# yanielc/medical-vision-textural-bias

Hardware: AMD Instinct MI355X
Metric: BraTS 4ch 240^3 vols/sec filtered+train-step @1/2/4/8 GPU; filter HBM GB/s (higher is better)
Workload: dtype f32

## Files before the change

medical-vision-textural-bias_amd/csrc/conv_wgrad.hip:

```cpp
#include <hip/hip_runtime.h>

#include <cstdlib>

#include "conv_host.h"
#include "split_bf16.h"
#include "texbias.h"

namespace {

typedef float f32x4 __attribute__((ext_vector_type(4)));

constexpr int NT = 256;
constexpr int LDS_FLOATS = 78 * 1024 / 4;
constexpr int kSlack = 16;

struct WgArgs {
  const float* G;
  const float* X;
  float* dW;
  int M, Cc, Do, Ho, Wo, Di, Hi, Wi;
  int YB, YR, Wo4, XP, PG, PC, ncc, ctiles, nyb, xcols;
  int64_t nchunks;
};

// ... 732 lines not shown
  }
#pragma unroll
  for (int j = 0; j < NGL; ++j) {
    const int i = tid + NT * j;
    const int q = i % Wo4, t = i / Wo4, yy = t % YB, m = t / YB;
    const bool ok = m < mv && y0 + yy < Ho;
    gg[j] = ok ? (int)(((int64_t)m * Do) * oplane / 4 + ((y0 + yy) * Wo + 4 * q) / 4) : -1;
    gl[j] = m * a.MS + yy * Wo + 4 * q;
  }
  const int64_t iplane4 = iplane / 4, oplane4 = oplane / 4;
  float4 rx0[NXL], rx1[NXL], rg[NGL];
  auto load_x = [&](int zi, float4 (&rx)[NXL]) {
    const bool in = zi >= 0 && zi < Di;
    const float4* src = reinterpret_cast<const float4*>(Xb) + (int64_t)(in ? zi : 0) * iplane4;
#pragma unroll
    for (int j = 0; j < NXL; ++j) rx[j] = src[xg[j] < 0 ? 0 : xg[j]];
  };
  auto store_x = [&](int zi, const float4 (&rx)[NXL]) {
    float* d = xsl + ((zi + 5) % 5) * XS;
    const bool in = zi >= 0 && zi < Di;
#pragma unroll
    for (int j = 0; j < NXL; ++j)
      if (xg[j] >= 0) {
        const float4 v = in ? rx[j] : make_float4(0.f, 0.f, 0.f, 0.f);
        float2* p = reinterpret_cast<float2*>(d + xl[j]);
        p[0] = make_float2(v.x, v.y);
        p[1] = make_float2(v.z, v.w);
      }
  };
  auto load_g = [&](int z) {
#pragma unroll
    for (int j = 0; j < NGL; ++j) {
      rg[j] = (reinterpret_cast<const float4*>(Gb) + (int64_t)z * oplane4)[gg[j] < 0 ? 0 : gg[j]];
    }
  };
  auto store_g = [&](int z) {
    float* d = gsl + (z & 1) * GS;
#pragma unroll
    for (int j = 0; j < NGL; ++j)
      if (gg[j] >= 0) {
        float2* p = reinterpret_cast<float2*>(d + gl[j]);
        p[0] = make_float2(rg[j].x, rg[j].y);
        p[1] = make_float2(rg[j].z, rg[j].w);
      }
  };
  __syncthreads();
  load_x(2 * z0 - 1, rx0);
  store_x(2 * z0 - 1, rx0);
  load_x(2 * z0, rx0);
  load_x(2 * z0 + 1, rx1);
  load_g(z0);

  const int li = lane & 15, lk = lane >> 4;
  const int mtl = wave & 1, par = wave >> 1;
  const int aoff = (16 * mtl + li) * a.MS + lk;
  const int boff = li * a.RX + 2 * lk + 1;
  f32x4 acc[27];
#pragma unroll
  for (int j = 0; j < 27; ++j) acc[j] = f32x4{0.f, 0.f, 0.f, 0.f};
  for (int z = z0; z < z1; ++z) {
    store_x(2 * z, rx0);
    store_x(2 * z + 1, rx1);
    store_g(z);
    __syncthreads();
    load_x(2 * z + 2, rx0);
    load_x(2 * z + 3, rx1);
    load_g(z + 1 < z1 ? z + 1 : z);
    const float* ga = gsl + (z & 1) * GS + aoff;
    const float* xp[3] = {xsl + ((2 * z - 1 + 5) % 5) * XS + boff, xsl + ((2 * z) % 5) * XS + boff,
                          xsl + ((2 * z + 1) % 5) * XS + boff};
    const int nk = YB * Wo4;
    auto ld = [&](int k, float& av, float (&bv)[27]) {
      const int kk = k < nk ? k : nk - 1;
      const int yy = YB == 1 ? 0 : (kk >= Wo4 ? 1 : 0), x0 = 4 * (kk - yy * Wo4);
      av = ga[yy * Wo + x0];
#pragma unroll
      for (int tz = 0; tz < 3; ++tz)
#pragma unroll
        for (int ty = 0; ty < 3; ++ty)
#pragma unroll
          for (int tx = 0; tx < 3; ++tx) bv[tz * 9 + ty * 3 + tx] = xp[tz][(2 * yy + ty) * a.PX + 2 * x0 + tx];
    };
    auto mm = [&](float av, const float (&bv)[27]) {
#pragma unroll
      for (int t = 0; t < 27; ++t) acc[t] = __builtin_amdgcn_mfma_f32_16x16x4f32(av, bv[t], acc[t], 0, 0, 0);
    };
    if (par < nk) {
      float a0, a1, b0[27], b1[27];
      ld(par, a0, b0);
      int k = par;
      for (; k + P < nk; k += 2 * P) {
        ld(k + P, a1, b1);
        mm(a0, b0);
        ld(k + 2 * P, a0, b0);
        mm(a1, b1);
      }
      if (k < nk) mm(a0, b0);
    }
  }
  float* red = smem;
#pragma unroll
  for (int src = P - 1; src >= 1; --src) {
    __syncthreads();
    if (par == src) {
#pragma unroll
      for (int j = 0; j < 27; ++j)
#pragma unroll
        for (int rr = 0; rr < 4; ++rr) red[((mtl * 27 + j) * 4 + rr) * 64 + lane] = acc[j][rr];
    }
    __syncthreads();
    if (par == 0) {
#pragma unroll
      for (int j = 0; j < 27; ++j)
#pragma unroll
        for (int rr = 0; rr < 4; ++rr) acc[j][rr] += red[((mtl * 27 + j) * 4 + rr) * 64 + lane];
    }
  }
  if (par == 0) {
    const int c = li;
    float* pt = a.part ? a.part + ((int64_t)blockIdx.y * gridDim.x + blockIdx.x) * (32 * 16 * 27) : nullptr;
#pragma unroll
    for (int j = 0; j < 27; ++j)
#pragma unroll
      for (int rr = 0; rr < 4; ++rr) {
        const int m = 16 * mtl + lk * 4 + rr;
        if (pt) pt[(m * 16 + c) * 27 + j] = acc[j][rr];
        else if (m < mv && c < cv) atomicAdd(&a.dW[((int64_t)(m0 + m) * a.Cc + (c0 + c)) * 27 + j], acc[j][rr]);
      }
  }
}


struct Zf2Args {
  const float* G;
  const float* X;
  float* dW;
  float* part;
  int N, M, Cc, Do, Ho, Wo, Di, Hi, Wi;
  int YB, nyb, ZS, zlen;
  int MS, RX, PX;
  int mtiles;
};

template <int YB, int MT, int WV, int NW>
__global__ __launch_bounds__(64 * NW) void k_conv3d_wgrad_zf2(Zf2Args a) {
  constexpr int NT = 64 * NW;
  constexpr int NXR = 2 * YB + 1;
  extern __shared__ __attribute__((aligned(16))) float smem[];
  const int tid = (int)threadIdx.x, lane = tid & 63;
  const int wave = __builtin_amdgcn_readfirstlane(tid >> 6);
  const int Wo = a.Wo, Ho = a.Ho, Do = a.Do, Hi = a.Hi, Wi = a.Wi, Di = a.Di, Cc = a.Cc;
  const int GS = 16 * MT * a.MS, XS = Cc * a.RX;
  float* gsl = smem;
  float* xsl = smem + 2 * GS;
  int b = (int)blockIdx.x;
  const int zs = b % a.ZS;
  b /= a.ZS;
  const int yb = b % a.nyb, n = b / a.nyb;
  const int mt = (int)blockIdx.y;
  const int m0 = 16 * MT * mt, mv = min(16 * MT, a.M - m0);
  const int y0 = yb * YB;
  const int z0 = zs * a.zlen, z1 = min(Do, z0 + a.zlen);
  for (int i = tid; i < 2 * GS + 5 * XS; i += NT) smem[i] = 0.f;
  const int64_t iplane = (int64_t)Hi * Wi, oplane = (int64_t)Ho * Wo;
  const float* Gb = a.G + ((int64_t)n * a.M + m0) * Do * oplane;
  const float* Xb = a.X + (int64_t)n * Cc * Di * iplane;
  const int Wi4 = Wi >> 2, Wo4 = Wo >> 2;
  constexpr int NXL = (5 * NXR * 2 * WV + NT - 1) / NT, NGL = (16 * MT * YB * WV + NT - 1) / NT;
  int xg[NXL], xl[NXL], gg[NGL], gl[NGL];
#pragma unroll
  for (int j = 0; j < NXL; ++j) {
    const int i = tid + NT * j;
    const int q = i % Wi4, t = i / Wi4, r = t % NXR, c = t / NXR;
    const int yi = 2 * y0 - 1 + r;
    const bool ok = c < Cc && yi >= 0 && yi < Hi;
    xg[j] = ok ? (int)(((int64_t)c * Di) * iplane / 4 + (yi * Wi + 4 * q) / 4) : -1;
    xl[j] = c * a.RX + r * a.PX + 2 + 4 * q;
  }
#pragma unroll
  for (int j = 0; j < NGL; ++j) {
    const int i = tid + NT * j;
    const int q = i % Wo4, t = i / Wo4, yy = t % YB, m = t / YB;
    const int y = y0 + yy;
    const bool ok = m < mv && y < Ho;
    gg[j] = ok ? (int)(((int64_t)m * Do) * oplane / 4 + (y * Wo + 4 * q) / 4) : -1;
    gl[j] = m * a.MS + yy * Wo + 4 * q;
  }
  const int64_t iplane4 = iplane / 4, oplane4 = oplane / 4;
  float4 rx0[NXL], rx1[NXL], rg[NGL];
  auto load_x = [&](int zi, float4 (&rx)[NXL]) {
    const bool in = zi >= 0 && zi < Di;
    const float4* src = reinterpret_cast<const float4*>(Xb) + (int64_t)(in ? zi : 0) * iplane4;
#pragma unroll
    for (int j = 0; j < NXL; ++j) rx[j] = src[xg[j] < 0 ? 0 : xg[j]];
  };
  auto store_x = [&](int zi, const float4 (&rx)[NXL]) {
    float* d = xsl + ((zi + 5) % 5) * XS;
    const bool in = zi >= 0 && zi < Di;
#pragma unroll
    for (int j = 0; j < NXL; ++j)
      if (xg[j] >= 0) {
        const float4 v = in ? rx[j] : make_float4(0.f, 0.f, 0.f, 0.f);
        float2* p = reinterpret_cast<float2*>(d + xl[j]);
        p[0] = make_float2(v.x, v.y);
        p[1] = make_float2(v.z, v.w);
      }
  };
  auto load_g = [&](int z) {
#pragma unroll
    for (int j = 0; j < NGL; ++j) {
      rg[j] = (reinterpret_cast<const float4*>(Gb) + (int64_t)z * oplane4)[gg[j] < 0 ? 0 : gg[j]];
    }
  };
  auto store_g = [&](int z) {
    float* d = gsl + (z & 1) * GS;
#pragma unroll
    for (int j = 0; j < NGL; ++j)
      if (gg[j] >= 0) {
        float2* p = reinterpret_cast<float2*>(d + gl[j]);
        p[0] = make_float2(rg[j].x, rg[j].y);
        p[1] = make_float2(rg[j].z, rg[j].w);
      }
  };
  __syncthreads();
  load_x(2 * z0 - 1, rx0);
  store_x(2 * z0 - 1, rx0);
  load_x(2 * z0, rx0);
  load_x(2 * z0 + 1, rx1);
  load_g(z0);

  const int li = lane & 15, lk = lane >> 4;
  const int bc = li < 3 * Cc ? li / 3 : 0, btx = li < 3 * Cc ? li - 3 * (li / 3) : 0;
  const int boff = bc * a.RX + btx + 2 * lk + 1;
  f32x4 acc[MT][9];
#pragma unroll
  for (int t = 0; t < MT; ++t)
#pragma unroll
    for (int j = 0; j < 9; ++j) acc[t][j] = f32x4{0.f, 0.f, 0.f, 0.f};
  for (int z = z0; z < z1; ++z) {
    store_x(2 * z, rx0);
    store_x(2 * z + 1, rx1);
    store_g(z);
    __syncthreads();
    load_x(2 * z + 2, rx0);
    load_x(2 * z + 3, rx1);
    load_g(z + 1 < z1 ? z + 1 : z);
    const float* ga = gsl + (z & 1) * GS + li * a.MS + lk;
    const float* xp[3] = {xsl + ((2 * z - 1 + 5) % 5) * XS + boff, xsl + ((2 * z) % 5) * XS + boff,
                          xsl + ((2 * z + 1) % 5) * XS + boff};
    const int np = YB >= NW ? 1 : NW / YB, yy0 = YB >= NW ? wave : wave % YB, part = YB >= NW ? 0 : wave / YB;
    const int kb = (Wo4 * part) / np, ke = (Wo4 * (part + 1)) / np;
    auto ld = [&](int yy, int k, float (&av)[MT], float (&bv)[9]) {
      const int x0 = 4 * (k < ke ? k : ke - 1);
#pragma unroll
      for (int t = 0; t < MT; ++t) av[t] = ga[t * 16 * a.MS + yy * Wo + x0];
#pragma unroll
      for (int tz = 0; tz < 3; ++tz)
#pragma unroll
        for (int ty = 0; ty < 3; ++ty) bv[tz * 3 + ty] = xp[tz][(2 * yy + ty) * a.PX + 2 * x0];
    };
    auto mm = [&](const float (&av)[MT], const float (&bv)[9]) {
#pragma unroll
      for (int t = 0; t < MT; ++t)
#pragma unroll
        for (int j = 0; j < 9; ++j) acc[t][j] = __builtin_amdgcn_mfma_f32_16x16x4f32(av[t], bv[j], acc[t][j], 0, 0, 0);
    };
    for (int yy = yy0; yy < YB; yy += NW) {
      if (kb >= ke) break;
      float a0[MT], a1[MT], b0[9], b1[9];
      ld(yy, kb, a0, b0);
      int k = kb;
      for (; k + 1 < ke; k += 2) {
        ld(yy, k + 1, a1, b1);
        mm(a0, b0);
        ld(yy, k + 2, a0, b0);
        mm(a1, b1);
      }
      if (k < ke) mm(a0, b0);
    }
  }
  __syncthreads();
  float* red = smem;
#pragma unroll
  for (int t = 0; t < MT; ++t)
#pragma unroll
    for (int j = 0; j < 9; ++j)
#pragma unroll
      for (int rr = 0; rr < 4; ++rr) red[(((t * 9 + j) * NW + wave) * 4 + rr) * 64 + lane] = acc[t][j][rr];
  __syncthreads();
  float* pt = a.part ? a.part + ((int64_t)blockIdx.y * gridDim.x + blockIdx.x) * (16 * MT * Cc * 27) : nullptr;
  for (int e = tid; e < MT * 9 * 4 * 64; e += NT) {
    const int ln = e & 63, rr = (e >> 6) & 3, tj = e >> 8, t = tj / 9, j = tj - 9 * t;
    const int m = 16 * t + (ln >> 4) * 4 + rr, col = ln & 15;
    if ((!pt && m >= mv) || col >= 3 * Cc) continue;
    float v = 0.f;
#pragma unroll
    for (int w = 0; w < NW; ++w) v += red[((tj * NW + w) * 4 + rr) * 64 + ln];
    const int c = col / 3, tx = col - 3 * c;
    if (pt) pt[(m * Cc + c) * 27 + j * 3 + tx] = v;
    else atomicAdd(&a.dW[((int64_t)(m0 + m) * Cc + c) * 27 + j * 3 + tx], v);
  }
}

struct Zf1Args {
  const float* G;
  const float* X;
  float* dW;
  float* part;
  double* bpart;
  int N, M, Cc, D, H, W;
  int YB, nyb, ZS, zlen;
  int GR, GM, GS;
  int XR, XC, XS;
};

constexpr size_t ZF1_RED_BYTES = (size_t)2 * 4 * 4 * 64 * 4;

template <int YB, int WV>
__global__ __launch_bounds__(256) void k_conv3d_wgrad_zf1(Zf1Args a) {
  extern __shared__ __attribute__((aligned(16))) float smem[];
  const int tid = (int)threadIdx.x, lane = tid & 63;
  const int wave = __builtin_amdgcn_readfirstlane(tid >> 6);
  const int W = a.W, H = a.H, D = a.D, M = a.M, Cc = a.Cc;
  float* gsl = smem;
  float* xsl = smem + 4 * a.GS;
  f32x4* smem4 = reinterpret_cast<f32x4*>(smem);
  const int dump = a.GS + (a.XS >> 1) + tid;
  int b = (int)blockIdx.x;
  const int zs = b % a.ZS;
  b /= a.ZS;
  const int yb = b % a.nyb, n = b / a.nyb;
  const int y0 = yb * YB;
  const int z0 = zs * a.zlen, z1 = min(D, z0 + a.zlen);
  for (int i = tid; i < 4 * a.GS + 2 * a.XS; i += 256) smem[i] = 0.f;
  const int64_t plane = (int64_t)H * W, plane4 = plane / 4;
  const float* Gb = a.G + (int64_t)n * M * D * plane;
  const float* Xb = a.X + (int64_t)n * Cc * D * plane;
  const int W4v = W >> 2;
  constexpr int NXL = (5 * YB * WV + 255) / 256, NGL = (3 * (YB + 2) * WV + 255) / 256;
  int xg[NXL], xl[NXL], gg[NGL], gl[NGL];
  bool own[NGL];
#pragma unroll
  for (int j = 0; j < NXL; ++j) {
    const int i = tid + 256 * j;
    const int q = i % W4v, t = i / W4v, yy = t % YB, c = t / YB;
    const bool ok = c < Cc && y0 + yy < H;
    xg[j] = ok ? (int)(((int64_t)c * D) * plane4 + ((y0 + yy) * W + 4 * q) / 4) : -1;
    xl[j] = ok ? a.GS + ((c * a.XC + yy * a.XR) >> 2) + 1 + q : dump;
  }
#pragma unroll
  for (int j = 0; j < NGL; ++j) {
    const int i = tid + 256 * j;
    const int q = i % W4v, t = i / W4v, r = t % (YB + 2), m = t / (YB + 2);
    const int y = y0 - 1 + r;
    const bool ok = m < M && y >= 0 && y < H;
    gg[j] = ok ? (int)(((int64_t)m * D) * plane4 + (y * W + 4 * q) / 4) : -1;
    gl[j] = ok ? ((m * a.GM + r * a.GR) >> 2) + q : dump;
    own[j] = ok && r >= 1 && r <= YB;
  }
  constexpr int ZP = 3;
  f32x4 rx0[NXL], rx1[NXL], rx2[NXL], rg0[NGL], rg1[NGL], rg2[NGL];
  double bs[NGL];
#pragma unroll
  for (int j = 0; j < NGL; ++j) bs[j] = 0.0;
  const bool bias = a.bpart != nullptr;
  auto load_x = [&](int zi, f32x4 (&r)[NXL]) {
    const f32x4* src = reinterpret_cast<const f32x4*>(Xb) + (int64_t)(zi < D ? zi : D - 1) * plane4;
#pragma unroll
    for (int j = 0; j < NXL; ++j) r[j] = src[xg[j] < 0 ? 0 : xg[j]];
  };
  auto store_x = [&](int slot, const f32x4 (&r)[NXL]) {
#pragma unroll
    for (int j = 0; j < NXL; ++j)
      smem4[(xg[j] >= 0 ? slot * (a.XS >> 2) : 0) + xl[j]] = r[j];
  };
  auto load_g = [&](int pz, f32x4 (&r)[NGL]) {
    const f32x4* src = reinterpret_cast<const f32x4*>(Gb) + (int64_t)(pz >= 0 && pz < D ? pz : 0) * plane4;
#pragma unroll
    for (int j = 0; j < NGL; ++j) r[j] = src[gg[j] < 0 ? 0 : gg[j]];
  };
  auto store_g = [&](int slot, const f32x4 (&r)[NGL], int pz) {
    const bool in = pz >= 0 && pz < D;
    const bool cnt = bias && pz >= z0 && pz < z1;
#pragma unroll
    for (int j = 0; j < NGL; ++j) {
      const f32x4 v = in ? r[j] : f32x4{0.f, 0.f, 0.f, 0.f};
      smem4[(gg[j] >= 0 ? slot * (a.GS >> 2) : 0) + gl[j]] = v;
      const float q = (v[0] + v[1]) + (v[2] + v[3]);
      bs[j] += (double)(own[j] && cnt ? q : 0.f);
    }
  };
  __syncthreads();
  load_g(z0 - 1, rg0);
  store_g((z0 + 3) & 3, rg0, z0 - 1);
  load_g(z0, rg0);
  store_g(z0 & 3, rg0, z0);
  load_x(z0, rx0);
  load_g(z0 + 1, rg0);
  load_x(z0 + 1, rx1);
  load_g(z0 + 2, rg1);
  load_x(z0 + 2, rx2);
  load_g(z0 + 3, rg2);
  const int li = lane & 15, lk = lane >> 4;
  int atz[2], aoff[2];
#pragma unroll
  for (int t = 0; t < 2; ++t) {
    const int r0 = 16 * t + li, r = r0 < 9 * M ? r0 : 0;
    const int m = r / 9, tz = (r / 3) % 3, ty = r % 3;
    atz[t] = tz;
    aoff[t] = m * a.GM + (2 - ty) * a.GR + 4 * lk;
  }
  const int col = li < 3 * Cc ? li : 0, bc = col / 3, btx = col - 3 * bc;
  const int boff = bc * a.XC + 3 + btx + 4 * lk;
  const int ngr = (W + 15) >> 4, np = 4 / YB, yy = wave % YB, part = wave / YB;
  const int gb = (ngr * part) / np, ge = (ngr * (part + 1)) / np;
  f32x4 acc[2][2];
#pragma unroll
  for (int t = 0; t < 2; ++t) acc[0][t] = acc[1][t] = f32x4{0.f, 0.f, 0.f, 0.f};
  auto mm = [&](const f32x4& v0, const f32x4& v1, const f32x4& u) {
#pragma unroll
    for (int s = 0; s < 4; ++s) {
      acc[s & 1][0] = __builtin_amdgcn_mfma_f32_16x16x4f32(v0[s], u[s], acc[s & 1][0], 0, 0, 0);
      acc[s & 1][1] = __builtin_amdgcn_mfma_f32_16x16x4f32(v1[s], u[s], acc[s & 1][1], 0, 0, 0);
    }
  };
  auto step = [&](int zi, f32x4 (&rxp)[NXL], f32x4 (&rgp)[NGL]) {
    store_x(zi & 1, rxp);
    store_g((zi + 1) & 3, rgp, zi + 1);
    __syncthreads();
    load_x(zi + ZP, rxp);
    load_g(zi + ZP + 1, rgp);
    const f32x4* ga0 = reinterpret_cast<const f32x4*>(gsl + ((zi + 1 - atz[0]) & 3) * a.GS + aoff[0] + yy * a.GR);
    const f32x4* ga1 = reinterpret_cast<const f32x4*>(gsl + ((zi + 1 - atz[1]) & 3) * a.GS + aoff[1] + yy * a.GR);
    const float* xb = xsl + (zi & 1) * a.XS + boff + yy * a.XR;
    auto ld = [&](int g, f32x4& v0, f32x4& v1, f32x4& u) {
      v0 = ga0[4 * g];
      v1 = ga1[4 * g];
      const float* p = xb + 16 * g;
      u = f32x4{p[0], p[1], p[2], p[3]};
    };
    if (gb < ge) {
      f32x4 p0, p1, pu, q0, q1, qu;
      ld(gb, p0, p1, pu);
      int g = gb;
      for (; g + 2 < ge; g += 2) {
        ld(g + 1, q0, q1, qu);
        __builtin_amdgcn_sched_barrier(0);
        mm(p0, p1, pu);
        __builtin_amdgcn_sched_barrier(0);
        ld(g + 2, p0, p1, pu);
        __builtin_amdgcn_sched_barrier(0);
        mm(q0, q1, qu);
        __builtin_amdgcn_sched_barrier(0);
      }
      if (g + 1 < ge) {
        ld(g + 1, q0, q1, qu);
        __builtin_amdgcn_sched_barrier(0);
        mm(p0, p1, pu);
        mm(q0, q1, qu);
      } else {
        mm(p0, p1, pu);
      }
    }
  };
  int zi = z0;
  for (; zi + ZP <= z1; zi += ZP) {
    step(zi, rx0, rg0);
    step(zi + 1, rx1, rg1);
    step(zi + 2, rx2, rg2);
  }
  if (zi < z1) {
    step(zi, rx0, rg0);
    if (zi + 1 < z1) step(zi + 1, rx1, rg1);
  }
  __syncthreads();
  float* red = smem;
#pragma unroll
  for (int t = 0; t < 2; ++t)
#pragma unroll
    for (int rr = 0; rr < 4; ++rr) red[((t * 4 + wave) * 4 + rr) * 64 + lane] = acc[0][t][rr] + acc[1][t][rr];
  double* bred = reinterpret_cast<double*>(reinterpret_cast<char*>(smem) + ZF1_RED_BYTES);
  if (bias) {
#pragma unroll
    for (int mm_ = 0; mm_ < 3; ++mm_) {
      double v = 0.0;
#pragma unroll
      for (int j = 0; j < NGL; ++j) v += ((tid + 256 * j) / W4v) / (YB + 2) == mm_ ? bs[j] : 0.0;
#pragma unroll
      for (int off = 32; off; off >>= 1) v += __shfl_down(v, off);
      if (lane == 0) bred[wave * 3 + mm_] = v;
    }
  }
  __syncthreads();
  if (bias && tid < M)
    a.bpart[(int64_t)blockIdx.x * M + tid] = (bred[tid] + bred[3 + tid]) + (bred[6 + tid] + bred[9 + tid]);
  float* pt = a.part ? a.part + (int64_t)blockIdx.x * (M * Cc * 27) : nullptr;
  for (int e = tid; e < 2 * 4 * 64; e += 256) {
    const int ln = e & 63, rr = (e >> 6) & 3, t = e >> 8;
    const int r = 16 * t + 4 * (ln >> 4) + rr, col = ln & 15;
    const int m = r / 9, c = col / 3;
    if (m >= M || c >= Cc) continue;
    const int tz = (r / 3) % 3, ty = r % 3, tx = col - 3 * c;
    const float v = red[((t * 4 + 0) * 4 + rr) * 64 + ln] + red[((t * 4 + 1) * 4 + rr) * 64 + ln] +
                    red[((t * 4 + 2) * 4 + rr) * 64 + ln] + red[((t * 4 + 3) * 4 + rr) * 64 + ln];
    if (pt) pt[(m * Cc + c) * 27 + tz * 9 + ty * 3 + tx] = v;
    else atomicAdd(&a.dW[((int64_t)m * Cc + c) * 27 + tz * 9 + ty * 3 + tx], v);
  }
}

int pad_mod(int v, int mod, int rem) {
  while (v % mod != rem) ++v;
  return v;
}

int pad_mod32(int v, int rem) {
  while ((v & 31) != rem) ++v;
  return v;
}

unsigned wg_grid_x(const WgArgs& a, int TX, int by) {
  int64_t gx = TX == 9 ? 1024 : (512 + by - 1) / by;
  if (gx > a.nchunks) gx = a.nchunks;
  return gx < 1 ? 1u : (unsigned)gx;
}

int launch_wg(const WgArgs& a, int stride, int TX, int seg, int by, size_t lds, hipStream_t st) {
  void (*kern)(WgArgs) = nullptr;
#define TB_WG(SEG)                                                                                             \
  case SEG:                                                                                                    \
    kern = TX == 9 ? k_conv3d_wgrad_mz<SEG>                                                                    \
                   : stride == 1 ? (TX == 1 ? k_conv3d_wgrad<1, 1, SEG> : k_conv3d_wgrad<1, 3, SEG>)            \
                                 : (TX == 1 ? k_conv3d_wgrad<2, 1, SEG> : k_conv3d_wgrad<2, 3, SEG>);            \
    break;
  switch (seg) {
    TB_WG(1) TB_WG(2) TB_WG(3) TB_WG(4)
    default: return TB_ERR_UNSUPPORTED_SIZE;
  }
#undef TB_WG
  return tb::launch_lds(kern, dim3(wg_grid_x(a, TX, by), (unsigned)by), dim3(NT), lds, st, a);
}

int wg_setup_mz(WgArgs& a, int& seg, int& by, size_t& lds, int N, int M, int Cc, int Do, int Ho, int Wo, int Di,
                int Hi, int Wi) {
  a.M = M; a.Cc = Cc; a.Do = Do; a.Ho = Ho; a.Wo = Wo; a.Di = Di; a.Hi = Hi; a.Wi = Wi;
  a.Wo4 = (Wo + 3) / 4 * 4;
  const int xw = a.Wo4 - 1 + 3;
  a.XP = xw | 1;
  a.xcols = Wi < a.XP - 1 ? Wi : a.XP - 1;
  seg = (((Wo > a.xcols ? Wo : a.xcols) + 63) / 64);
  if (seg > 4) return TB_ERR_UNSUPPORTED_SIZE;
  a.YB = 0;
  constexpr int yb_max = 4;
  for (int yb : {8, 4, 2, 1}) {
    if ((yb > 1 && yb > Ho) || yb > yb_max) continue;
    const int yr = yb + 2;
    const int pg = pad_mod32(yb * a.Wo4, 2);
    const int pc = pad_mod32(yr * a.XP, 3);
    if (3 * M * pg + Cc * pc + kSlack <= LDS_FLOATS) {
      a.YB = yb; a.YR = yr; a.PG = pg; a.PC = pc;
      break;
    }
  }
  if (!a.YB) return TB_ERR_UNSUPPORTED_SIZE;
  a.nyb = (Ho + a.YB - 1) / a.YB;
  a.nchunks = (int64_t)N * Di * a.nyb;
  const int carve = 3 * M * a.PG + Cc * a.PC + kSlack;
  lds = sizeof(float) * (size_t)(carve > 4 * 3 * 4 * 64 ? carve : 4 * 3 * 4 * 64);
  by = 1;
  return TB_OK;
}

bool use_mz(int M, int Cc, int stride) { return stride == 1 && M <= 5 && Cc <= 5; }

int wg_setup(WgArgs& a, int& seg, int& TX, int& by, size_t& lds, int N, int M, int Cc, int Do, int Ho, int Wo, int Di,
             int Hi, int Wi, int stride, int pad) {
  if (N < 1 || M < 1 || Cc < 1 || Do < 1 || Ho < 1 || Wo < 1 || Di < 1 || Hi < 1 || Wi < 1) return TB_ERR_INVALID_ARG;
  if ((stride != 1 && stride != 2) || pad != 1) return TB_ERR_INVALID_ARG;
  if (use_mz(M, Cc, stride)) {
    TX = 9;
    return wg_setup_mz(a, seg, by, lds, N, M, Cc, Do, Ho, Wo, Di, Hi, Wi);
  }
  a.M = M; a.Cc = Cc; a.Do = Do; a.Ho = Ho; a.Wo = Wo; a.Di = Di; a.Hi = Hi; a.Wi = Wi;
  TX = Cc <= 5 ? 3 : 1;
  a.ncc = TX == 3 ? 5 : 16;
  a.Wo4 = (Wo + 3) / 4 * 4;
  const int xw = stride * (a.Wo4 - 1) + 3;
  a.XP = xw | 1;
  a.xcols = Wi < a.XP - 1 ? Wi : a.XP - 1;
  seg = (((Wo > a.xcols ? Wo : a.xcols) + 63) / 64);
  if (seg > 4) return TB_ERR_UNSUPPORTED_SIZE;
  const int prem = TX == 3 ? 3 : 2;
  a.YB = 0;
  constexpr int yb_max = 8;
  for (int yb : {8, 4, 2, 1}) {
    if ((yb > 1 && yb > Ho) || yb > yb_max) continue;
    const int yr = stride * (yb - 1) + 3;
    const int pg = pad_mod32(yb * a.Wo4, 2);
    const int pc = pad_mod32(3 * yr * a.XP, prem);
    if ((M < 16 ? M : 16) * pg + (Cc < a.ncc ? Cc : a.ncc) * pc + kSlack <= LDS_FLOATS) {
      a.YB = yb; a.YR = yr; a.PG = pg; a.PC = pc;
      break;
    }
  }
  if (!a.YB) return TB_ERR_UNSUPPORTED_SIZE;
  a.nyb = (Ho + a.YB - 1) / a.YB;
  a.nchunks = (int64_t)N * Do * a.nyb;
  const int mtiles = (M + 15) / 16;
  a.ctiles = (Cc + a.ncc - 1) / a.ncc;
  lds = sizeof(float) * (size_t)((M < 16 ? M : 16) * a.PG + (Cc < a.ncc ? Cc : a.ncc) * a.PC + kSlack);
  by = mtiles * a.ctiles;
  return TB_OK;
}


bool use_zm(int M, int Cc, int stride, int Do, int Ho, int Wo, int Di, int Hi, int Wi) {
  return stride == 1 && M >= 8 && Cc >= 8 && Do == Di && Ho == Hi && Wo == Wi && Wo % 4 == 0 && Wo <= 80;
}

int zm_setup(ZmArgs& a, size_t& lds, dim3& grid, int N, int M, int Cc, int D, int H, int W) {
  a.N = N; a.M = M; a.Cc = Cc; a.D = D; a.H = H; a.W = W;
  a.W4 = W;
  a.PX = ((W + 3 + 1) / 2) * 2;
  a.YB = 0;
  for (int yb : {4, 2}) {
    const int ms = pad_mod32(yb * a.W4, 2), rx = pad_mod32((yb + 2) * a.PX, 2);
    const size_t bytes = (size_t)4 * (4 * 16 * ms + 2 * 16 * rx);
    if (bytes <= 163840) {
      a.YB = yb; a.MS = ms; a.RX = rx;
      lds = bytes > ZM_RED_BYTES ? bytes : ZM_RED_BYTES;
      if (lds < 81920 + 16) lds = 81920 + 16;
      break;
    }
  }
  if (!a.YB) return TB_ERR_UNSUPPORTED_SIZE;
  a.nyb = (H + a.YB - 1) / a.YB;
  a.mtiles = (M + 15) / 16;
  a.ctiles = (Cc + 15) / 16;
  a.zlen = tb::zseg(D, N * a.nyb * a.mtiles * a.ctiles, 1, 2, 4);
  a.ZS = (D + a.zlen - 1) / a.zlen;
  grid = dim3((unsigned)(N * a.nyb * a.ZS), (unsigned)(a.mtiles * a.ctiles));
  return TB_OK;
}

bool zm_split(const ZmArgs& a) { return a.YB == 4 && a.W != 12 && a.W != 20; }

int launch_zm(const ZmArgs& a, size_t lds, dim3 grid, hipStream_t st) {
  if (zm_split(a)) {
    auto kern = a.W % 8 == 0 ? (a.W > 40 ? k_conv3d_wgrad_zm_split<4, 20, true> : k_conv3d_wgrad_zm_split<4, 10, true>)
                             : (a.W > 40 ? k_conv3d_wgrad_zm_split<4, 20, false> : k_conv3d_wgrad_zm_split<4, 10, false>);
    return tb::launch_lds(kern, grid, dim3(768), lds, st, a);
  }
  auto kern = a.W > 40 ? (a.YB == 4 ? k_conv3d_wgrad_zm<4, 20, 8> : k_conv3d_wgrad_zm<2, 20, 8>)
                       : (a.YB == 4 ? k_conv3d_wgrad_zm<4, 10, 8> : k_conv3d_wgrad_zm<2, 10, 8>);
  return tb::launch_lds(kern, grid, dim3(512), lds, st, a);
}

bool use_zm2(int M, int Cc, int stride, int Do, int Ho, int Wo, int Di, int Hi, int Wi) {
  return stride == 2 && M >= 8 && Cc >= 8 && Wo % 4 == 0 && Wo <= 40 && Wi == 2 * Wo && Hi == 2 * Ho && Di == 2 * Do;
}

int zm2_setup(Zm2Args& a, size_t& lds, dim3& grid, int N, int M, int Cc, int Do, int Ho, int Wo, int Di, int Hi,
              int Wi) {
  a.N = N; a.M = M; a.Cc = Cc; a.Do = Do; a.Ho = Ho; a.Wo = Wo; a.Di = Di; a.Hi = Hi; a.Wi = Wi;
  a.PX = ((2 * Wo + 3 + 1) / 2) * 2;
  a.YB = 0;
  for (int yb : {2, 1}) {
    if (yb > Ho) continue;
    for (int rem : {2, 4}) {
      const int rx = pad_mod32((2 * yb + 1) * a.PX, rem), ms = pad_mod32(yb * Wo, 2);
      const size_t ring = (size_t)4 * (2 * 32 * ms + 5 * 16 * rx), red = (size_t)4 * 2 * 27 * 4 * 64;
      const size_t need = ring > red ? ring : red;
      if (need <= 163840) {
        a.YB = yb; a.RX = rx; a.MS = ms;
        lds = need;
        break;
      }
    }
    if (a.YB) break;
  }
  if (!a.YB) return TB_ERR_UNSUPPORTED_SIZE;
  a.nyb = (Ho + a.YB - 1) / a.YB;
  a.mtiles = (M + 31) / 32;
  a.ctiles = (Cc + 15) / 16;
  a.zlen = tb::zseg(Do, N * a.nyb * a.mtiles * a.ctiles, 1, 1);
  a.ZS = (Do + a.zlen - 1) / a.zlen;
  grid = dim3((unsigned)(N * a.nyb * a.ZS), (unsigned)(a.mtiles * a.ctiles));
  return TB_OK;
}

int launch_zm2(const Zm2Args& a, size_t lds, dim3 grid, hipStream_t st) {
  auto kern = a.YB == 2 ? (a.Wo <= 20 ? k_conv3d_wgrad_zm2<2, 5, 8> : k_conv3d_wgrad_zm2<2, 10, 8>)
                        : (a.Wo <= 20 ? k_conv3d_wgrad_zm2<1, 5, 8> : k_conv3d_wgrad_zm2<1, 10, 8>);
  return tb::launch_lds(kern, grid, dim3(512), lds, st, a);
}

bool use_zf2(int M, int Cc, int stride, int Do, int Ho, int Wo, int Di, int Hi, int Wi) {
  return stride == 2 && Cc <= 5 && Wo % 4 == 0 && Wo <= 80 && Wi == 2 * Wo && Hi == 2 * Ho && Di == 2 * Do;
}

int zf2_setup(Zf2Args& a, int& MT, size_t& lds, dim3& grid, int N, int M, int Cc, int Do, int Ho, int Wo, int Di,
              int Hi, int Wi) {
  a.N = N; a.M = M; a.Cc = Cc; a.Do = Do; a.Ho = Ho; a.Wo = Wo; a.Di = Di; a.Hi = Hi; a.Wi = Wi;
  MT = M > 16 ? 2 : 1;
  a.PX = ((2 * Wo + 3 + 1) / 2) * 2;
  a.YB = 0;
  for (int yb : {4, 2, 1}) {
    const int rx = pad_mod32((2 * yb + 1) * a.PX, 8), ms = pad_mod32(yb * Wo, 2);
    const size_t ring = (size_t)4 * (2 * 16 * MT * ms + 5 * Cc * rx), red = (size_t)4 * MT * 9 * 8 * 4 * 64;
    const size_t need = ring > red ? ring : red;
    if (need <= 163840) {
      a.YB = yb; a.RX = rx; a.MS = ms;
      lds = need;
      break;
    }
  }
  if (!a.YB) return TB_ERR_UNSUPPORTED_SIZE;
  a.nyb = (Ho + a.YB - 1) / a.YB;
  a.mtiles = (M + 16 * MT - 1) / (16 * MT);
  a.zlen = tb::zseg(Do, N * a.nyb * a.mtiles, 1, 1);
  a.ZS = (Do + a.zlen - 1) / a.zlen;
  grid = dim3((unsigned)(N * a.nyb * a.ZS), (unsigned)a.mtiles);
  return TB_OK;
}

template <int YB, int MT>
auto zf2_kern(int Wo) {
  return Wo <= 40 ? k_conv3d_wgrad_zf2<YB, MT, 10, 8> : k_conv3d_wgrad_zf2<YB, MT, 20, 8>;
}
int launch_zf2(const Zf2Args& a, int MT, size_t lds, dim3 grid, hipStream_t st) {
  auto kern = MT == 1 ? (a.YB == 4 ? zf2_kern<4, 1>(a.Wo) : a.YB == 2 ? zf2_kern<2, 1>(a.Wo) : zf2_kern<1, 1>(a.Wo))
                      : (a.YB == 4 ? zf2_kern<4, 2>(a.Wo) : a.YB == 2 ? zf2_kern<2, 2>(a.Wo) : zf2_kern<1, 2>(a.Wo));
  return tb::launch_lds(kern, grid, dim3(512), lds, st, a);
}

bool use_zf1(int M, int Cc, int stride, int Do, int Ho, int Wo, int Di, int Hi, int Wi) {
  return stride == 1 && M <= 3 && Cc <= 5 && Do == Di && Ho == Hi && Wo == Wi && Wo % 4 == 0 && Wo <= 256;
}

int zf1_setup(Zf1Args& a, size_t& lds, dim3& grid, int N, int M, int Cc, int D, int H, int W) {
  a.N = N; a.M = M; a.Cc = Cc; a.D = D; a.H = H; a.W = W;
  const int Wp = (W + 15) & ~15;
  a.GR = pad_mod(Wp, 64, 40);
  a.XR = pad_mod32(Wp + 8, 4);
  a.YB = 0;
  for (int yb : {2, 4, 1}) {
    const int gm = pad_mod((yb + 2) * a.GR, 64, 24), gs = pad_mod(M * gm, 64, 56);
    const int xc = pad_mod32(yb * a.XR, 8), xs = pad_mod32(Cc * xc, 16);
    const size_t bytes = (size_t)4 * (4 * gs + 2 * xs + 4 * 256);
    if (bytes <= 81920) {
      a.YB = yb; a.GM = gm; a.GS = gs; a.XC = xc; a.XS = xs;
      const size_t red = ZF1_RED_BYTES + 4 * 3 * sizeof(double);
      lds = bytes > red ? bytes : red;
      break;
    }
  }
  if (!a.YB) return TB_ERR_UNSUPPORTED_SIZE;
  a.nyb = (H + a.YB - 1) / a.YB;
  a.zlen = tb::zseg(D, N * a.nyb, 2, 2);
  a.ZS = (D + a.zlen - 1) / a.zlen;
  grid = dim3((unsigned)(N * a.nyb * a.ZS));
  return TB_OK;
}

template <int YB>
auto zf1_kern(int W) {
  return W <= 128 ? k_conv3d_wgrad_zf1<YB, 32> : W <= 160 ? k_conv3d_wgrad_zf1<YB, 40> : k_conv3d_wgrad_zf1<YB, 64>;
}
int launch_zf1(const Zf1Args& a, size_t lds, dim3 grid, hipStream_t st) {
  auto kern = a.YB == 4 ? zf1_kern<4>(a.W) : a.YB == 2 ? zf1_kern<2>(a.W) : zf1_kern<1>(a.W);
  return tb::launch_lds(kern, grid, dim3(256), lds, st, a);
}

struct ZRoute {
  int kind = 0;
  ZmArgs zm{};
  Zm2Args zm2{};
  Zf1Args zf1{};
  Zf2Args zf2{};
  int MT = 1;
  size_t lds = 0;
  dim3 grid;
  int TM = 0, TC = 0, ctiles = 1;
  int YB = 0, zlen = 0, ZS = 0;
  size_t bytes() const { return kind ? (size_t)grid.x * grid.y * TM * TC * 27 * 4 : 0; }
  template <class A>
  void take(int k, const A& a, int tm, int tc, int ct) {
    kind = k, TM = tm, TC = tc, ctiles = ct, YB = a.YB, zlen = a.zlen, ZS = a.ZS;
  }
};

bool aligned16(const void* G, const void* X) {
  return ((reinterpret_cast<uintptr_t>(G) | reinterpret_cast<uintptr_t>(X)) & 15) == 0;
}

ZRoute zroute(int N, int M, int Cc, int Do, int Ho, int Wo, int Di, int Hi, int Wi, int stride, int pad,
              bool aligned = true) {
  ZRoute r;
  if (pad != 1 || N < 1 || !aligned) return r;
  if (use_zm(M, Cc, stride, Do, Ho, Wo, Di, Hi, Wi) && zm_setup(r.zm, r.lds, r.grid, N, M, Cc, Do, Ho, Wo) == TB_OK)
    r.take(1, r.zm, 16, 16, r.zm.ctiles);
  else if (use_zm2(M, Cc, stride, Do, Ho, Wo, Di, Hi, Wi) &&
           zm2_setup(r.zm2, r.lds, r.grid, N, M, Cc, Do, Ho, Wo, Di, Hi, Wi) == TB_OK)
    r.take(2, r.zm2, 32, 16, r.zm2.ctiles);
  else if (use_zf1(M, Cc, stride, Do, Ho, Wo, Di, Hi, Wi) &&
           zf1_setup(r.zf1, r.lds, r.grid, N, M, Cc, Do, Ho, Wo) == TB_OK)
    r.take(3, r.zf1, M, Cc, 1);
  else if (use_zf2(M, Cc, stride, Do, Ho, Wo, Di, Hi, Wi) &&
           zf2_setup(r.zf2, r.MT, r.lds, r.grid, N, M, Cc, Do, Ho, Wo, Di, Hi, Wi) == TB_OK)
    r.take(4, r.zf2, 16 * r.MT, Cc, 1);
  return r;
}

template <class A>
const A& bound(A& a, const float* G, const float* X, float* dW, float* part) {
  a.G = G, a.X = X, a.dW = dW, a.part = part;
  return a;
}

int zrun(ZRoute& r, const float* G, const float* X, float* dW, float* part, double* bpart, hipStream_t st) {
  switch (r.kind) {
    case 1: return launch_zm(bound(r.zm, G, X, dW, part), r.lds, r.grid, st);
    case 2: return launch_zm2(bound(r.zm2, G, X, dW, part), r.lds, r.grid, st);
    case 3: r.zf1.bpart = bpart; return launch_zf1(bound(r.zf1, G, X, dW, part), r.lds, r.grid, st);
    default: return launch_zf2(bound(r.zf2, G, X, dW, part), r.MT, r.lds, r.grid, st);
  }
}
}

int tb_conv3d_wgrad_f32(const float* G, const float* X, float* dW, int N, int M, int Cc, int Do, int Ho, int Wo, int Di,
                        int Hi, int Wi, int stride, int pad, void* stream) {
  if (!G || !X || !dW) return TB_ERR_INVALID_ARG;
  hipStream_t st = reinterpret_cast<hipStream_t>(stream);
  ZRoute r = zroute(N, M, Cc, Do, Ho, Wo, Di, Hi, Wi, stride, pad, aligned16(G, X));
  WgArgs a{};
  int seg = 0, TX = 0, by = 0;
  size_t lds = 0;
  if (!r.kind) {
    const int rc = wg_setup(a, seg, TX, by, lds, N, M, Cc, Do, Ho, Wo, Di, Hi, Wi, stride, pad);
    if (rc != TB_OK) return rc;
  }
  if (hipMemsetAsync(dW, 0, sizeof(float) * (size_t)M * Cc * 27, st) != hipSuccess) return TB_ERR_HIP;
  if (r.kind) return zrun(r, G, X, dW, nullptr, nullptr, st);
  a.G = G; a.X = X; a.dW = dW;
  return launch_wg(a, stride, TX, seg, by, lds, st);
}

int64_t tb_conv3d_wgrad_ws_bytes(int N, int M, int Cc, int Do, int Ho, int Wo, int Di, int Hi, int Wi, int stride,
                                 int pad) {
  return (int64_t)zroute(N, M, Cc, Do, Ho, Wo, Di, Hi, Wi, stride, pad).bytes();
}

static size_t bias_off(const ZRoute& r) { return (r.bytes() + 7) & ~(size_t)7; }
static size_t bias_bytes(const ZRoute& r, int M) { return r.kind == 3 ? (size_t)r.grid.x * M * sizeof(double) : 0; }

int64_t tb_conv3d_wgrad_bias_ws_bytes(int N, int M, int Cc, int Do, int Ho, int Wo, int Di, int Hi, int Wi, int stride,
                                      int pad, int* sums_bias) {
  const ZRoute r = zroute(N, M, Cc, Do, Ho, Wo, Di, Hi, Wi, stride, pad);
  const size_t bb = bias_bytes(r, M);
  if (sums_bias) *sums_bias = bb ? 1 : 0;
  return (int64_t)(bb ? bias_off(r) + bb : r.bytes());
}

int tb_conv3d_wgrad_bias_ws_f32(const float* G, const float* X, float* dW, float* dbias, int N, int M, int Cc, int Do,
                                int Ho, int Wo, int Di, int Hi, int Wi, int stride, int pad, void* ws, size_t ws_bytes,
                                int* bias_done, void* stream) {
  if (bias_done) *bias_done = 0;
  if (!G || !X || !dW) return TB_ERR_INVALID_ARG;
  hipStream_t st = reinterpret_cast<hipStream_t>(stream);
  ZRoute r = zroute(N, M, Cc, Do, Ho, Wo, Di, Hi, Wi, stride, pad, aligned16(G, X));
  if (!ws || !r.kind || ws_bytes < r.bytes() || (reinterpret_cast<uintptr_t>(ws) & 3) != 0)
    return tb_conv3d_wgrad_f32(G, X, dW, N, M, Cc, Do, Ho, Wo, Di, Hi, Wi, stride, pad, stream);
  float* part = static_cast<float*>(ws);
  double* bpart = nullptr;
  if (dbias && bias_bytes(r, M) && ws_bytes >= bias_off(r) + bias_bytes(r, M) &&
      (reinterpret_cast<uintptr_t>(ws) & 7) == 0)
    bpart = reinterpret_cast<double*>(static_cast<char*>(ws) + bias_off(r));
  const int rc = zrun(r, G, X, dW, part, bpart, st);
  if (rc != TB_OK) return rc;
  hipLaunchKernelGGL(k_wgrad_reduce, dim3((r.TM * r.TC * 27 + 63) / 64 + (bpart ? 1 : 0), r.grid.y), dim3(1024), 0, st,
                     static_cast<const float*>(part), dW, (int)r.grid.x, r.TM, r.TC, r.ctiles, M, Cc,
                     static_cast<const double*>(bpart), dbias);
  if (hipGetLastError() != hipSuccess) return TB_ERR_HIP;
  if (bias_done) *bias_done = bpart ? 1 : 0;
  return TB_OK;
}

int tb_conv3d_wgrad_ws_f32(const float* G, const float* X, float* dW, int N, int M, int Cc, int Do, int Ho, int Wo,
                           int Di, int Hi, int Wi, int stride, int pad, void* ws, size_t ws_bytes, void* stream) {
  return tb_conv3d_wgrad_bias_ws_f32(G, X, dW, nullptr, N, M, Cc, Do, Ho, Wo, Di, Hi, Wi, stride, pad, ws, ws_bytes,
                                     nullptr, stream);
}

int tb_conv3d_wgrad_config(int N, int M, int Cc, int Do, int Ho, int Wo, int Di, int Hi, int Wi, int stride, int pad,
                           int64_t* cfg) {
  if (!cfg) return TB_ERR_INVALID_ARG;
  WgArgs a{};
  int seg = 0, TX = 0, by = 0;
  size_t lds = 0;
  const int rc = wg_setup(a, seg, TX, by, lds, N, M, Cc, Do, Ho, Wo, Di, Hi, Wi, stride, pad);
  if (rc != TB_OK) return rc;
  cfg[0] = seg; cfg[1] = TX; cfg[2] = a.YB; cfg[3] = a.nchunks; cfg[4] = (int64_t)lds;
  return TB_OK;
}

int tb_conv3d_wgrad_plan(int N, int M, int Cc, int Do, int Ho, int Wo, int Di, int Hi, int Wi, int stride, int pad,
                         int64_t* cfg) {
  if (!cfg) return TB_ERR_INVALID_ARG;
  const ZRoute r = zroute(N, M, Cc, Do, Ho, Wo, Di, Hi, Wi, stride, pad);
  WgArgs a{};
  int seg = 0, TX = 0, by = 0;
  size_t lds = r.lds;
  if (!r.kind) {
    const int rc = wg_setup(a, seg, TX, by, lds, N, M, Cc, Do, Ho, Wo, Di, Hi, Wi, stride, pad);
    if (rc != TB_OK) return rc;
  }
  cfg[0] = r.kind; cfg[1] = r.kind ? r.YB : a.YB; cfg[2] = r.zlen; cfg[3] = r.ZS;
  cfg[4] = r.kind ? r.grid.x : wg_grid_x(a, TX, by); cfg[5] = r.kind ? r.grid.y : (unsigned)by;
  cfg[6] = (int64_t)lds; cfg[7] = (int64_t)r.bytes();
  return TB_OK;
}
```

Baseline: 200.0.

## Add 768-thread split-tap variant of stride-2 wgrad kernel for selected widths

Adds a 768-thread variant of the stride-2 zf2 weight-gradient kernel. The 12 waves are split as 3 z-taps by 4 phases, so each wave accumulates only one z-tap's 3 y-taps instead of all nine, with a FULL specialization that drops bounds checks when the work divides evenly. It is selected by a width heuristic (overridable through an env var) for YB>=2 and particular Wo values. The aim is more parallelism per block and fewer accumulator registers. The cost is higher LDS pressure per block, possibly lower occupancy, and a cross-wave reduction at the end.

```diff
diff --git a/medical-vision-textural-bias_amd/csrc/conv_wgrad.hip b/medical-vision-textural-bias_amd/csrc/conv_wgrad.hip
--- a/medical-vision-textural-bias_amd/csrc/conv_wgrad.hip
+++ b/medical-vision-textural-bias_amd/csrc/conv_wgrad.hip
@@ -1058,6 +1058,182 @@
   }
 }
 
+template <int YB, int MT, int WV, bool FULL>
+__global__ __launch_bounds__(768) void k_conv3d_wgrad_zf2_split(Zf2Args a) {
+  constexpr int NT = 768;
+  constexpr int NXR = 2 * YB + 1;
+  extern __shared__ __attribute__((aligned(16))) float smem[];
+  const int tid = (int)threadIdx.x, lane = tid & 63;
+  const int wave = __builtin_amdgcn_readfirstlane(tid >> 6);
+  const int Wo = a.Wo, Ho = a.Ho, Do = a.Do, Hi = a.Hi, Wi = a.Wi, Di = a.Di, Cc = a.Cc;
+  const int GS = 16 * MT * a.MS, XS = Cc * a.RX;
+  float* gsl = smem;
+  float* xsl = smem + 2 * GS;
+  int b = (int)blockIdx.x;
+  const int zs = b % a.ZS;
+  b /= a.ZS;
+  const int yb = b % a.nyb, n = b / a.nyb;
+  const int mt = (int)blockIdx.y;
+  const int m0 = 16 * MT * mt, mv = min(16 * MT, a.M - m0);
+  const int y0 = yb * YB;
+  const int z0 = zs * a.zlen, z1 = min(Do, z0 + a.zlen);
+  for (int i = tid; i < 2 * GS + 5 * XS; i += NT) smem[i] = 0.f;
+  const int64_t iplane = (int64_t)Hi * Wi, oplane = (int64_t)Ho * Wo;
+  const float* Gb = a.G + ((int64_t)n * a.M + m0) * Do * oplane;
+  const float* Xb = a.X + (int64_t)n * Cc * Di * iplane;
+  const int Wi4 = Wi >> 2, Wo4 = Wo >> 2;
+  constexpr int NXL = (5 * NXR * 2 * WV + NT - 1) / NT, NGL = (16 * MT * YB * WV + NT - 1) / NT;
+  int xg[NXL], xl[NXL], gg[NGL], gl[NGL];
+#pragma unroll
+  for (int j = 0; j < NXL; ++j) {
+    const int i = tid + NT * j;
+    const int q = i % Wi4, t = i / Wi4, r = t % NXR, c = t / NXR;
+    const int yi = 2 * y0 - 1 + r;
+    const bool ok = c < Cc && yi >= 0 && yi < Hi;
+    xg[j] = ok ? (int)(((int64_t)c * Di) * iplane / 4 + (yi * Wi + 4 * q) / 4) : -1;
+    xl[j] = c * a.RX + r * a.PX + 2 + 4 * q;
+  }
+#pragma unroll
+  for (int j = 0; j < NGL; ++j) {
+    const int i = tid + NT * j;
+    const int q = i % Wo4, t = i / Wo4, yy = t % YB, m = t / YB;
+    const int y = y0 + yy;
+    const bool ok = m < mv && y < Ho;
+    gg[j] = ok ? (int)(((int64_t)m * Do) * oplane / 4 + (y * Wo + 4 * q) / 4) : -1;
+    gl[j] = m * a.MS + yy * Wo + 4 * q;
+  }
+  const int64_t iplane4 = iplane / 4, oplane4 = oplane / 4;
+  float4 rx0[NXL], rx1[NXL], rg[NGL];
+  auto load_x = [&](int zi, float4 (&rx)[NXL]) {
+    const bool in = zi >= 0 && zi < Di;
+    const float4* src = reinterpret_cast<const float4*>(Xb) + (int64_t)(in ? zi : 0) * iplane4;
+#pragma unroll
+    for (int j = 0; j < NXL; ++j) rx[j] = src[xg[j] < 0 ? 0 : xg[j]];
+  };
+  auto store_x = [&](int zi, const float4 (&rx)[NXL]) {
+    float* d = xsl + ((zi + 5) % 5) * XS;
+    const bool in = zi >= 0 && zi < Di;
+#pragma unroll
+    for (int j = 0; j < NXL; ++j)
+      if (xg[j] >= 0) {
+        const float4 v = in ? rx[j] : make_float4(0.f, 0.f, 0.f, 0.f);
+        float2* p = reinterpret_cast<float2*>(d + xl[j]);
+        p[0] = make_float2(v.x, v.y);
+        p[1] = make_float2(v.z, v.w);
+      }
+  };
+  auto load_g = [&](int z) {
+#pragma unroll
+    for (int j = 0; j < NGL; ++j) {
+      rg[j] = (reinterpret_cast<const float4*>(Gb) + (int64_t)z * oplane4)[gg[j] < 0 ? 0 : gg[j]];
+    }
+  };
+  auto store_g = [&](int z) {
+    float* d = gsl + (z & 1) * GS;
+#pragma unroll
+    for (int j = 0; j < NGL; ++j)
+      if (gg[j] >= 0) {
+        float2* p = reinterpret_cast<float2*>(d + gl[j]);
+        p[0] = make_float2(rg[j].x, rg[j].y);
+        p[1] = make_float2(rg[j].z, rg[j].w);
+      }
+  };
+  __syncthreads();
+  load_x(2 * z0 - 1, rx0);
+  store_x(2 * z0 - 1, rx0);
+  load_x(2 * z0, rx0);
+  load_x(2 * z0 + 1, rx1);
+  load_g(z0);
+
+  const int li = lane & 15, lk = lane >> 4;
+  const int tz = wave % 3, ph = wave / 3;
+  const int bc = li < 3 * Cc ? li / 3 : 0, btx = li < 3 * Cc ? li - 3 * (li / 3) : 0;
+  const int boff = bc * a.RX + btx + 1;
+  const int GPR = (Wo + 7) >> 3, NG = YB * GPR, nsteps = (NG + 3) >> 2;
+  tb::f32x4s hi[MT][3], lo[MT][3];
+#pragma unroll
+  for (int t = 0; t < MT; ++t)
+#pragma unroll
+    for (int j = 0; j < 3; ++j) hi[t][j] = lo[t][j] = tb::f32x4s{0.f, 0.f, 0.f, 0.f};
+  auto step = [&](const float* ga, const float* xp, int s) {
+    const int g = 4 * s + lk;
+    const bool in = FULL || g < NG;
+    const int gc = in ? g : 0;
+    int yy = 0;
+#pragma unroll
+    for (int r = 1; r < YB; ++r) yy += gc >= r * GPR ? 1 : 0;
+    const int x0 = 8 * (gc - yy * GPR);
+    const int nv = !in ? 0 : min(8, Wo - x0);
+    tb::bf16x8 af[MT][3];
+#pragma unroll
+    for (int t = 0; t < MT; ++t) {
+      const float2* src = reinterpret_cast<const float2*>(ga + t * 16 * a.MS + yy * Wo + x0);
+      float v[8];
+#pragma unroll
+      for (int i = 0; i < 4; ++i) {
+        const float2 u = src[i];
+        v[2 * i] = u.x;
+        v[2 * i + 1] = u.y;
+      }
+      tb::split3(v, af[t][0], af[t][1], af[t][2]);
+    }
+#pragma unroll
+    for (int ty = 0; ty < 3; ++ty) {
+      const float* xr = xp + (2 * yy + ty) * a.PX + 2 * x0;
+      float v[8];
+#pragma unroll
+      for (int j = 0; j < 8; ++j) {
+        if constexpr (FULL) {
+          v[j] = xr[2 * j];
+        } else {
+          const float u = xr[2 * max(min(j, nv - 1), 0)];
+          v[j] = j < nv ? u : 0.f;
+        }
+      }
+      tb::bf16x8 bf[3];
+      tb::split3(v, bf[0], bf[1], bf[2]);
+#pragma unroll
+      for (int t = 0; t < MT; ++t) tb::mfma_split6(af[t], bf, hi[t][ty], lo[t][ty]);
+    }
+  };
+  int s = ph;
+  for (int z = z0; z < z1; ++z) {
+    store_x(2 * z, rx0);
+    store_x(2 * z + 1, rx1);
+    store_g(z);
+    __syncthreads();
+    load_x(2 * z + 2, rx0);
+    load_x(2 * z + 3, rx1);
+    load_g(z + 1 < z1 ? z + 1 : z);
+    const float* ga = gsl + (z & 1) * GS + li * a.MS;
+    const float* xp = xsl + ((2 * z - 1 + tz + 5) % 5) * XS + boff;
+    for (; s < nsteps; s += 4) step(ga, xp, s);
+    s -= nsteps;
+  }
+  __syncthreads();
+  float* red = smem;
+#pragma unroll
+  for (int t = 0; t < MT; ++t)
+#pragma unroll
+    for (int ty = 0; ty < 3; ++ty)
+#pragma unroll
+      for (int rr = 0; rr < 4; ++rr)
+        red[(((t * 9 + tz * 3 + ty) * 4 + ph) * 4 + rr) * 64 + lane] = hi[t][ty][rr] + lo[t][ty][rr];
+  __syncthreads();
+  float* pt = a.part ? a.part + ((int64_t)blockIdx.y * gridDim.x + blockIdx.x) * (16 * MT * Cc * 27) : nullptr;
+  for (int e = tid; e < MT * 9 * 4 * 64; e += NT) {
+    const int ln = e & 63, rr = (e >> 6) & 3, tj = e >> 8, t = tj / 9, j = tj - 9 * t;
+    const int m = 16 * t + (ln >> 4) * 4 + rr, col = ln & 15;
+    if ((!pt && m >= mv) || col >= 3 * Cc) continue;
+    float v = 0.f;
+#pragma unroll
+    for (int w = 0; w < 4; ++w) v += red[((tj * 4 + w) * 4 + rr) * 64 + ln];
+    const int c = col / 3, tx = col - 3 * c;
+    if (pt) pt[(m * Cc + c) * 27 + j * 3 + tx] = v;
+    else atomicAdd(&a.dW[((int64_t)(m0 + m) * Cc + c) * 27 + j * 3 + tx], v);
+  }
+}
+
 struct Zf1Args {
   const float* G;
   const float* X;
@@ -1483,7 +1659,41 @@
 auto zf2_kern(int Wo) {
   return Wo <= 40 ? k_conv3d_wgrad_zf2<YB, MT, 10, 8> : k_conv3d_wgrad_zf2<YB, MT, 20, 8>;
 }
+int s2_split_forced() {
+  static const int v = [] {
+    const char* e = std::getenv("TEXBIAS_WGRAD_S2_SPLIT");
+    return e && (e[0] == '0' || e[0] == '1') ? e[0] - '0' : -1;
+  }();
+  return v;
+}
+
+bool zf2_split(const Zf2Args& a, int MT) {
+  if (a.YB < 2 || (a.YB == 4 && MT == 2 && a.Wo > 40)) return false;
+  if (s2_split_forced() >= 0) return s2_split_forced() == 1;
+  const int Wo = a.Wo;
+  if (MT == 2) return (Wo >= 32 && Wo <= 40) || Wo == 80;
+  return (Wo >= 32 && Wo <= 40) || Wo == 48 || Wo >= 72;
+}
+
+template <int YB, int MT>
+auto zf2_split_kern(int Wo) {
+  const bool full = Wo % 8 == 0 && (YB * (Wo / 8)) % 4 == 0;
+  if constexpr (YB == 2) {
+    return full ? k_conv3d_wgrad_zf2_split<YB, MT, 20, true> : k_conv3d_wgrad_zf2_split<YB, MT, 20, false>;
+  } else if constexpr (MT == 2) {
+    return full ? k_conv3d_wgrad_zf2_split<YB, MT, 10, true> : k_conv3d_wgrad_zf2_split<YB, MT, 10, false>;
+  } else {
+    return full ? (Wo <= 40 ? k_conv3d_wgrad_zf2_split<YB, MT, 10, true> : k_conv3d_wgrad_zf2_split<YB, MT, 20, true>)
+                : (Wo <= 40 ? k_conv3d_wgrad_zf2_split<YB, MT, 10, false> : k_conv3d_wgrad_zf2_split<YB, MT, 20, false>);
+  }
+}
+
 int launch_zf2(const Zf2Args& a, int MT, size_t lds, dim3 grid, hipStream_t st) {
+  if (zf2_split(a, MT)) {
+    auto kern = MT == 1 ? (a.YB == 4 ? zf2_split_kern<4, 1>(a.Wo) : zf2_split_kern<2, 1>(a.Wo))
+                        : (a.YB == 4 ? zf2_split_kern<4, 2>(a.Wo) : zf2_split_kern<2, 2>(a.Wo));
+    return tb::launch_lds(kern, grid, dim3(768), lds, st, a);
+  }
   auto kern = MT == 1 ? (a.YB == 4 ? zf2_kern<4, 1>(a.Wo) : a.YB == 2 ? zf2_kern<2, 1>(a.Wo) : zf2_kern<1, 1>(a.Wo))
                       : (a.YB == 4 ? zf2_kern<4, 2>(a.Wo) : a.YB == 2 ? zf2_kern<2, 2>(a.Wo) : zf2_kern<1, 2>(a.Wo));
   return tb::launch_lds(kern, grid, dim3(512), lds, st, a);
```

Measured after the change: 200.5 (median of 6 runs). No clear change (+0.3%).
